# ka9q/ka9q-radio

Hardware: NVIDIA H100
Metric: input Msamples/s through forward+filter+inverse at N channels (higher is better)
Workload: dtype f32

## Files before the change

include/ka9q_gpu.h:

```cpp
#ifndef KA9Q_GPU_H
#define KA9Q_GPU_H 1
#include <stddef.h>
#include <stdint.h>

#ifdef __cplusplus
extern "C" {
#endif

enum kgpu_type { KGPU_COMPLEX = 1, KGPU_REAL = 2 };
enum kgpu_format {
  KGPU_FMT_F32 = 0,
  KGPU_FMT_I16 = 1
};
enum kgpu_chan_flags {
  KGPU_CHAN_ISB = 1,
  KGPU_CHAN_BEAM = 4
};

typedef struct kgpu_master kgpu_master;
typedef struct kgpu_bank kgpu_bank;

struct kgpu_ingest_stats {
  unsigned long long energy;
  unsigned int clips;
// ... 132 lines not shown
long kgpu_bank_out_offset(kgpu_bank const *b, int idx);
int kgpu_bank_run(kgpu_bank *b, const void *d_spec, int nblocks, void *d_out, void *stream);
int kgpu_bank_run_ex(kgpu_bank *b, const void *d_spec, int nblocks, void *d_out, long out_pitch, float *d_power, void *stream);
int kgpu_bank_run_one(kgpu_bank *b, int idx, const void *d_spec, void *d_out, void *stream);
int kgpu_bank_run_one_ex(kgpu_bank *b, int idx, const void *d_spec, void *d_out, float *d_power , void *stream);
int kgpu_bank_noise(kgpu_bank *b, const void *d_spec, int nblocks, double samprate, double *d_n0, void *stream);

int kgpu_bank_fm_front(kgpu_bank *b, const void *d_out, long out_pitch, int nblocks, float *d_baseband, double *d_stats, void *stream);

int kgpu_bank_commit(kgpu_bank *b, void *stream);
int kgpu_use_static_kernels(int on);
int kgpu_use_cols_tma(int on);
int kgpu_cols_tma_fits(int L, int M, int in_type, int fmt, const void *d_in);
int kgpu_use_fused_forward(int on);
int kgpu_fused_forward_fits(int L, int M, int in_type, int fmt, const void *d_in);
int kgpu_fused_forward_options(int lead, int discard);
int kgpu_fused_shape(int *out);
int kgpu_fused_schedule(int nblocks, int lead, int ticket, int *out);
long kgpu_fused_discards(int blk, int idx, long *lines, long max);

int kgpu_plan_radices(int len, int *radices, int max);
int kgpu_plan_split(long n, int *n1, int *n2);
int kgpu_plan_radices_ex(int len, int *radices, int max);
int kgpu_plan_split_ex(long n, int *n1, int *n2);

int kgpu_multicast_copy(const void *d_src, void *mc_dst, unsigned long long bytes, int nctas, void *stream);

typedef struct kgpu_spectrum kgpu_spectrum;
kgpu_spectrum *kgpu_spectrum_create(int fft_n, int in_type, int bin_count);
int kgpu_spectrum_set_window(kgpu_spectrum *s, float const *window);
int kgpu_spectrum_run(kgpu_spectrum *s, const void *d_ring, long ring_samples, long end, int fmt, float scale,
                      const struct kgpu_scale_change *d_chg, int nchg, long long end_index, int derandomize, int shift, int fft_avg, double overlap, float *d_bins, void *stream);
int kgpu_spectrum_run_narrow(kgpu_spectrum *s, const void *d_ring, long ring_size, long ring_idx, int fft_avg,
                             double overlap, float *d_bins, int *fft_avg_used, void *stream);
// ... 12 lines not shown
```

ka9q_radio_b200/capi.py:

```python
from __future__ import annotations

import ctypes as C
import os
import subprocess
from pathlib import Path

PKG = Path(__file__).resolve().parent
LIB_PATH = PKG / "libka9qgpu.so"

KGPU_COMPLEX, KGPU_REAL = 1, 2
KGPU_FMT_F32, KGPU_FMT_I16 = 0, 1
KGPU_RAW_U8, KGPU_RAW_S8 = 1, 2
KGPU_RAW_S16, KGPU_RAW_U16, KGPU_RAW_SC16Q11 = 3, 4, 5
KGPU_RAW_F32, KGPU_RAW_CF32, KGPU_RAW_CF32_CNRMF, KGPU_RAW_CF32_FSCALE = 6, 7, 8, 9
KGPU_CHAN_ISB = 1
KGPU_CHAN_BEAM = 4

_lib = None


class KgpuError(RuntimeError):
    pass


# ... 81 lines not shown
    L.kgpu_bank_block_counter.restype = l
    L.kgpu_bank_run_ex.argtypes = [vp, vp, i, vp, l, vp, vp]
    L.kgpu_bank_run_one_ex.argtypes = [vp, i, vp, vp, vp, vp]
    L.kgpu_bank_noise.argtypes = [vp, vp, i, d, vp, vp]
    L.kgpu_bank_fm_front.argtypes = [vp, vp, l, i, vp, vp, vp]
    L.kgpu_use_static_kernels.argtypes = [i]
    L.kgpu_use_cols_tma.argtypes = [i]
    L.kgpu_cols_tma_fits.argtypes = [i, i, i, i, vp]
    L.kgpu_use_fused_forward.argtypes = [i]
    L.kgpu_fused_forward_fits.argtypes = [i, i, i, i, vp]
    L.kgpu_fused_forward_options.argtypes = [i, i]
    L.kgpu_fused_shape.argtypes = [vp]
    L.kgpu_fused_schedule.argtypes = [i, i, i, vp]
    L.kgpu_fused_discards.argtypes = [i, i, vp, l]
    L.kgpu_fused_discards.restype = l
    L.kgpu_profile_enable.argtypes = [i]
    L.kgpu_profile_name.argtypes = [i]
    L.kgpu_profile_name.restype = C.c_char_p
    L.kgpu_profile_get.argtypes = [i, vp, vp]
    L.kgpu_plan_radices.argtypes = [i, vp, i]
    L.kgpu_plan_split.argtypes = [l, vp, vp]
    L.kgpu_plan_radices_ex.argtypes = [i, vp, i]
    L.kgpu_plan_split_ex.argtypes = [l, vp, vp]
    L.kgpu_multicast_copy.argtypes = [vp, vp, C.c_ulonglong, i, vp]
    L.kgpu_algorithmic_bytes.argtypes = [vp, vp, i]
    L.kgpu_algorithmic_bytes.restype = d
    L.kgpu_spectrum_create.restype = vp
    L.kgpu_spectrum_create.argtypes = [i, i, i]
    L.kgpu_spectrum_set_window.argtypes = [vp, vp]
    L.kgpu_spectrum_run.argtypes = [vp, vp, l, l, i, f, vp, i, C.c_longlong, i, i, i, d, vp, vp]
# ... 369 lines not shown
```

ka9q_radio_b200/csrc/fft_static.cuh:

```cuda
#pragma once
#include "fft_radix.cuh"

namespace kfft {

template <int LEN, int... RS> struct SPlan {
  static constexpr int len = LEN;
  static constexpr int nst = sizeof...(RS);
  static constexpr int rad_arr[sizeof...(RS) > 0 ? sizeof...(RS) : 1] = {RS...};
  static constexpr int rad(int i) { return rad_arr[i]; }
  static constexpr int nsub(int i) {
    int n = LEN;
    for (int k = 0; k < i; k++) n /= rad_arr[k];
    return n;
  }
  static constexpr int stride(int i) { return nsub(i) / rad_arr[i]; }
  static constexpr int tw_off(int i) {
    int o = 0;
    for (int k = 0; k < i; k++)
      if (stride(k) > 1) o += (rad_arr[k] - 1) * stride(k);
    return o;
  }
  static constexpr bool valid() {
    int p = 1;
    for (int k = 0; k < nst; k++) p *= rad_arr[k];
// ... 99 lines not shown
};

__device__ __forceinline__ uint32_t smem_u32(void const *p) { return (uint32_t)__cvta_generic_to_shared(p); }
__device__ __forceinline__ void mbar_init(uint64_t *bar, int count) {
  asm volatile("mbarrier.init.shared::cta.b64 [%0], %1;" ::"r"(smem_u32(bar)), "r"(count));
}
__device__ __forceinline__ void mbar_fence_init() { asm volatile("fence.mbarrier_init.release.cluster;" ::: "memory"); }
__device__ __forceinline__ void mbar_expect_tx(uint64_t *bar, uint32_t bytes) {
  asm volatile("mbarrier.arrive.expect_tx.shared::cta.b64 _, [%0], %1;" ::"r"(smem_u32(bar)), "r"(bytes) : "memory");
}
__device__ __forceinline__ void bulk_g2s(void *dst, void const *src, uint32_t bytes, uint64_t *bar) {
  asm volatile("cp.async.bulk.shared::cluster.global.mbarrier::complete_tx::bytes [%0], [%1], %2, [%3];" ::"r"(smem_u32(dst)),
               "l"(src), "r"(bytes), "r"(smem_u32(bar))
               : "memory");
}
__device__ __forceinline__ void tensor_g2s_3d(void *dst, void const *map, int x, int y, int z, uint64_t *bar) {
  asm volatile("cp.async.bulk.tensor.3d.shared::cluster.global.tile.mbarrier::complete_tx::bytes [%0], [%1, {%2, %3, %4}], [%5];"
               ::"r"(smem_u32(dst)), "l"(map), "r"(x), "r"(y), "r"(z), "r"(smem_u32(bar))
               : "memory");
}
__device__ __forceinline__ void fence_proxy_async_global() { asm volatile("fence.proxy.async.global;" ::: "memory"); }
__device__ __forceinline__ void discard_l2_line(void *p) { asm volatile("discard.global.L2 [%0], 128;" ::"l"(p) : "memory"); }
__device__ __forceinline__ void mbar_wait(uint64_t *bar, uint32_t parity) {
  asm volatile(
      "{\n\t.reg .pred p;\n\t"
      "WAIT_%=:\n\t"
      "mbarrier.try_wait.parity.shared::cta.b64 p, [%0], %1;\n\t"
      "@p bra DONE_%=;\n\t"
      "bra WAIT_%=;\n\t"
      "DONE_%=:\n\t}" ::"r"(smem_u32(bar)),
// ... 6 lines not shown
```

ka9q_radio_b200/csrc/fwd_fused.cuh:

```cuda
#pragma once
#include "fwd_cols_r36.cuh"
#include "static_kernels_v2.cuh"

namespace kfft {

struct FusedShape {
  static constexpr int N1 = 1296, N2 = 1250;
  static constexpr int TILES = (N2 + 7) / 8;
  static constexpr int NC = (TILES + 1) / 2;
  static constexpr int NR = (N1 / 2 + 1 + RowsV2Shape<true>::IPC - 1) / RowsV2Shape<true>::IPC;
  static constexpr int T = 2 * ColsR36Shape::T;
  static constexpr int RT = RowsV2Shape<true>::T;
  static constexpr size_t smem = 2 * ColsR36Shape::smem > RowsV2Shape<true>::smem ? 2 * ColsR36Shape::smem : RowsV2Shape<true>::smem;
  static constexpr int DEFAULT_LEAD = 40;
  static_assert(ColsR36Shape::smem % 16 == 0, "the second tile's memory 16-byte aligned");
  static_assert(T % 32 == 0 && ColsR36Shape::T % 32 == 0 && RT % 32 == 0, "whole warps per tile and per R item");
};

enum FusedKind : int { kFusedCol = 0, kFusedRow = 1 };
struct FusedItem {
  int kind, blk, idx;
};

__host__ __device__ __forceinline__ FusedItem fused_item(int t, int nblocks, int lead) {
// ... 12 lines not shown
  unsigned *ctr;
  int nblocks, lead;
  int discard;
};

__device__ __forceinline__ void red_release_gpu_add(unsigned *p, unsigned v) {
  asm volatile("red.release.gpu.global.add.u32 [%0], %1;" ::"l"(p), "r"(v) : "memory");
}
__device__ __forceinline__ unsigned ld_acquire_gpu(unsigned const *p) {
  unsigned v;
  asm volatile("ld.acquire.gpu.global.u32 %0, [%1];" : "=r"(v) : "l"(p) : "memory");
  return v;
}

template <int FMT>
__global__ void __launch_bounds__(FusedShape::T, 1)
    fwd_fused_r36_v2(Pass1Args const a1, ColsR36Tables const t1, Pass2Args const a2, FwdTables const t2, FusedArgs const f,
                     const __grid_constant__ CUtensorMap tmap) {
  using F = FusedShape;
  extern __shared__ __align__(16) unsigned char smem_raw[];
  __shared__ __align__(8) uint64_t bars[RowsV2Shape<true>::COLS];
  __shared__ __align__(8) uint64_t tbar[2];
  __shared__ int s_ticket;
  int const tid = threadIdx.x;
  if (tid == 0) s_ticket = (int)atomicAdd(f.ctr, 1u);
  __syncthreads();
  FusedItem const it = fused_item(s_ticket, f.nblocks, f.lead);
  if (it.kind == kFusedCol) {
    int const h = tid >= ColsR36Shape::T, tile = 2 * it.idx + h;
    if (tile < F::TILES)
      fwd_cols_r36_body<FMT, F::N2, true>(a1, t1, &tmap, smem_raw + h * ColsR36Shape::smem, tbar[h], tid - h * ColsR36Shape::T,
                                           tile * 8, it.blk, [h] {
                                             asm volatile("bar.sync %0, %1;" ::"r"(1 + h), "n"(ColsR36Shape::T) : "memory");
                                           });
    __syncthreads();
    if (tid == 0) {
      __threadfence();
      red_release_gpu_add(f.ctr + 1 + fused_item(s_ticket, f.nblocks, f.lead).blk, 1u);
    }
    return;
  }
  if (tid >= F::RT) return;
  auto sync = [] { asm volatile("bar.sync 3, %0;" ::"n"(F::RT) : "memory"); };
  auto sync_or = [](int p) {
    int r;
    asm volatile("{\n\t.reg .pred q, o;\n\tsetp.ne.s32 q, %1, 0;\n\tbar.red.or.pred o, 3, %2, q;\n\tselp.s32 %0, 1, 0, o;\n\t}"
                 : "=r"(r)
                 : "r"(p), "n"(F::RT)
                 : "memory");
    return r;
  };
  if (tid == 0)
    while (ld_acquire_gpu(f.ctr + 1 + it.blk) < (unsigned)F::NC) __nanosleep(64);
  sync();
  fwd_rows_v2_body<true, F::N1, true, true>(a2, t2, smem_raw, bars, tbar[0], tid, it.blk, it.idx * RowsV2Shape<true>::IPC,
                                            sync, sync_or, f.discard);
}

}
```

ka9q_radio_b200/csrc/kgpu.cu:

```cuda
#include <cuda_runtime.h>
#include <cudaTypedefs.h>
#include <math.h>
#include <stdarg.h>
#include <stdio.h>
#include <stdlib.h>
#include <string.h>
#include <algorithm>
#include <complex>
#include <atomic>
#include <map>
#include <mutex>
#include <string>
#include <vector>

#include "../../include/ka9q_gpu.h"
#include "chan_kernels.cuh"
#include "chan_huge.cuh"
#include "chan_wide.cuh"
#include "fwd_kernels.cuh"
#include "noise_kernel.cuh"
#include "plan.cuh"
#include "static_kernels.cuh"
#include "static_kernels_v2.cuh"
#include "fwd_cols_r36.cuh"
// ... 19 lines not shown
static std::atomic<int> g_cols_tma{-1};
extern "C" int kgpu_use_cols_tma(int on) {
  g_cols_tma.store(on != 0);
  return 0;
}
static bool cols_tma_on() {
  int v = g_cols_tma.load();
  if (v < 0) {
    char const *e = getenv("KA9Q_COLS_TMA");
    g_cols_tma.compare_exchange_strong(v, (e && *e) ? (atoi(e) != 0) : 1);
    v = g_cols_tma.load();
  }
  return v != 0;
}
static std::atomic<int> g_fused{-1};
static std::atomic<int> g_fused_lead{FusedShape::DEFAULT_LEAD}, g_fused_discard{0};
extern "C" int kgpu_use_fused_forward(int on) {
  g_fused.store(on != 0);
  return 0;
}
static bool fused_on() {
  int v = g_fused.load();
  if (v < 0) {
    char const *e = getenv("KA9Q_FUSED_FWD");
    g_fused.compare_exchange_strong(v, (e && *e) ? (atoi(e) != 0) : 1);
    v = g_fused.load();
  }
  return v != 0;
}

static int fail(char const *fmt, ...) {
  char buf[512];
  va_list ap;
  va_start(ap, fmt);
  vsnprintf(buf, sizeof buf, fmt, ap);
  va_end(ap);
  g_err = buf;
  return -1;
}
#define CUDA_OK(expr)                                                                    \
  do {                                                                                   \
    cudaError_t e_ = (expr);                                                             \
    if (e_ != cudaSuccess) return fail("%s: %s (%s:%d)", #expr, cudaGetErrorString(e_), __FILE__, __LINE__); \
// ... 921 lines not shown
  return k[f];
}
static RowsV2Fn rows_v2_kernel(kgpu_master const *m) {
  if (m->in_type == KGPU_REAL) return m->halved ? fwd_rows_v2<true, 1296, true> : fwd_rows_v2<true, 0, false>;
  return m->n1c ? fwd_rows_v2<false, 1296, false> : fwd_rows_v2<false, 0, false>;
}
static bool fused_pair(kgpu_master const *m) {
  return m->in_type == KGPU_REAL && m->cols == COLS_R36 && m->rows == ROWS_V2 && m->halved && m->n2c == FusedShape::N2 &&
         m->n1c == FusedShape::N1 && m->mid_ld % 16 == 0;
}
using FusedFn = void (*)(Pass1Args, ColsR36Tables, Pass2Args, FwdTables, FusedArgs, CUtensorMap);
static FusedFn fused_kernel(int f) {
  static FusedFn const k[3] = {fwd_fused_r36_v2<0>, fwd_fused_r36_v2<1>, fwd_fused_r36_v2<2>};
  return k[f];
}
static int rows_v2_threads(kgpu_master const *m) { return m->in_type == KGPU_REAL ? RowsV2Shape<true>::T : RowsV2Shape<false>::T; }
static size_t rows_v2_smem(kgpu_master const *m) {
  return m->in_type == KGPU_REAL ? RowsV2Shape<true>::smem : RowsV2Shape<false>::smem;
}

static int upload(float2 **d, std::vector<float2> const &v) {
  CUDA_OK(cudaMalloc(d, sizeof(float2) * v.size()));
  CUDA_OK(cudaMemcpy(*d, v.data(), sizeof(float2) * v.size(), cudaMemcpyHostToDevice));
  return 0;
}

static int bluestein_upload(Bluestein *b) {
  if (upload(&b->d_b, bluestein_bspec(b->n, b->P)) == 0) return 0;
  cudaFree(b->d_b);
  b->d_b = nullptr;
// ... 84 lines not shown
      for (int j = 0; j < RB; j++) t0[(size_t)e * RB + j] = root((long)j * Pow<RA>::exponent(e), n1);
    for (long c = 0; c < n2; c++) {
      for (int t = 0; t < RA; t++) tA[(size_t)c * RA + t] = root(c * t, m->nc);
      for (int e = 0; e < Cols2s::NP1; e++) tB[(size_t)c * Cols2s::NP1 + e] = root(c * RA * Pow<RB>::exponent(e), m->nc);
    }
    for (int e = 0; e < Rows2s::NP0; e++)
      for (int j = 0; j < RD; j++) r0[(size_t)e * RD + j] = root((long)j * Pow<RC>::exponent(e), n2);
    if (upload(&m->d_tw0, t0) || upload(&m->d_twA, tA) || upload(&m->d_twB, tB) || upload(&m->d_rtw0, r0)) return -1;
    for (int f = 0; f < 3; f++)
      if (allow_smem((const void *)cols_2s_kernel(f), Cols2s::smem)) return -1;
    if (allow_smem((const void *)fwd_rows_2s<25, 25>, Rows2s::smem)) return -1;
  }
  if (m->rows == ROWS_V2 && allow_smem((const void *)rows_v2_kernel(m), rows_v2_smem(m))) return -1;
  if (fused_pair(m))
    for (int f = 0; f < 3; f++)
      if (allow_smem((const void *)fused_kernel(f), FusedShape::smem)) return -1;
  if (m->ext) {
    if (allow_smem((const void *)fwd_cols_ext<0>, m->smem1) || allow_smem((const void *)fwd_cols_ext<1>, m->smem1) ||
        allow_smem((const void *)fwd_rows_ext, m->smem2))
      return -1;
  } else if (allow_smem((const void *)fwd_cols_kernel<0>, m->smem1) || allow_smem((const void *)fwd_cols_kernel<1>, m->smem1) ||
             allow_smem((const void *)fwd_rows_kernel, m->smem2)) {
    return -1;
  }
  return 0;
}

extern "C" void kgpu_master_destroy(kgpu_master *m) {
  if (!m) return;
  if (m->ext) {
    free_tile_plan(m->xplan1);
// ... 193 lines not shown
  MasterPlan pl;
  if (master_plan(L, M, in_type, MP_BLUESTEIN, "kgpu_fused_forward_fits", &pl)) return -1;
  if (pl.path != MP_DIRECT) return 0;
  kgpu_master m;
  master_shape(&m, L, M, in_type, pl.sp, false);
  return fused_fits(&m, d_in, fmt) ? 1 : 0;
}

extern "C" int kgpu_fused_forward_options(int lead, int discard) {
  if (lead < 0 || lead > FusedShape::NC) return fail("kgpu_fused_forward_options: lead %d outside 0..%d", lead, FusedShape::NC);
  g_fused_lead.store(lead);
  g_fused_discard.store(discard != 0);
  return 0;
}

extern "C" int kgpu_fused_shape(int *out) {
  if (!out) return fail("kgpu_fused_shape: bad arguments");
  out[0] = FusedShape::NC;
  out[1] = FusedShape::NR;
  out[2] = FusedShape::N1;
  out[3] = (FusedShape::N2 + 15) / 16 * 16;
  out[4] = FusedShape::DEFAULT_LEAD;
  return 0;
}

extern "C" int kgpu_fused_schedule(int nblocks, int lead, int ticket, int *out) {
  if (nblocks < 1 || lead < 0 || lead > FusedShape::NC || ticket < 0 || ticket >= nblocks * (FusedShape::NC + FusedShape::NR) ||
      !out)
    return fail("kgpu_fused_schedule: bad arguments");
  FusedItem const it = fused_item(ticket, nblocks, lead);
  out[0] = it.kind;
  out[1] = it.blk;
  out[2] = it.idx;
  out[3] = it.kind == kFusedRow ? it.blk : -1;
  out[4] = it.kind == kFusedRow ? FusedShape::NC : 0;
  return 0;
}

extern "C" long kgpu_fused_discards(int blk, int idx, long *lines, long max) {
  using S = RowsV2Shape<true>;
  if (blk < 0 || idx < 0 || idx >= FusedShape::NR || max < 0) return fail("kgpu_fused_discards: bad arguments");
  int const ld = (FusedShape::N2 + 15) / 16 * 16;
  long n = 0;
  for (int col = 0; col < S::COLS; col++) {
    RowItem const it = row_item(idx * S::IPC + (col >> 1), FusedShape::N1, true);
    int const row = (col & 1) == 0 ? (it.kind != kRowEmpty ? it.row_a : -1) : (it.kind == kRowPair ? it.row_b : -1);
    if (row < 0) continue;
    for (int l = 0; l < mid_row_lines(ld); l++, n++)
      if (lines && n < max) lines[n] = mid_line(blk, FusedShape::N1, row, ld, l);
  }
  return n;
// ... 30 lines not shown
  a2.n2 = m->sp.n2;
  a2.nc = m->nc;
  a2.plan = m->plan2;
  a2.pitch = m->pitch2;
  a2.real_split = (m->in_type == KGPU_REAL);
  a2.rootD = m->d_rootD;
  a2.spec = (float2 *)d_spec;
  a2.spec_stride = m->spec_stride;
  a2.mid_ld = a1.mid_ld;
  return a2;
}

static int fused_span(kgpu_master *m, const void *d_in, int fmt, int f, int nblocks, void *d_spec, cudaStream_t st,
                      Pass1Args const &a1) {
  using F = FusedShape;
  size_t const ctr_bytes = sizeof(unsigned) * (size_t)(1 + nblocks);
  if (grow(m->fused_ctr, ctr_bytes, st, "kgpu_forward")) return -1;
  CUtensorMap map;
  if (cols_tma_map(m, d_in, fmt, nblocks, &map)) return -1;
  FusedArgs fa;
  fa.ctr = (unsigned *)m->fused_ctr.p;
  fa.nblocks = nblocks;
  fa.lead = g_fused_lead.load();
  fa.discard = g_fused_discard.load();
  CUDA_OK(cudaMemsetAsync(fa.ctr, 0, ctr_bytes, st));
  {
    ProfScope ps(K_FWD_FUSED, st);
    fused_kernel(f)<<<(unsigned)(nblocks * (F::NC + F::NR)), F::T, F::smem, st>>>(a1, ColsR36Tables{m->d_tw0, m->d_twA, m->d_twB},
                                                                       rows_args(m, a1, d_spec), FwdTables{m->d_rootC}, fa, map);
  }
  g_launches++;
  CUDA_OK(cudaGetLastError());
  return 0;
}

static int forward_span(kgpu_master *m, const void *d_in, int fmt, float scale, int derandomize, int nblocks, void *d_spec,
                        void *d_stats, cudaStream_t st, float2 *mid) {
  bool const use_static = g_static_on.load() != 0;
  ColsKernel const cols = use_static ? m->cols : COLS_GENERIC;
  RowsKernel const rows = use_static ? m->rows : ROWS_GENERIC;
  Pass1Args a1;
  a1.in = d_in;
  a1.hop = (m->in_type == KGPU_REAL) ? m->L / 2 : m->L;
  a1.n1 = m->sp.n1;
// ... 1399 lines not shown
```

ka9q_radio_b200/csrc/static_kernels_v2.cuh:

```cuda
#pragma once
#include "static_kernels.cuh"

namespace kfft {

__device__ __forceinline__ void unpack_i16(int raw, int &lo, int &hi) {
  asm("prmt.b32 %0, %1, 0, 0x9910;" : "=r"(lo) : "r"(raw));
  hi = raw >> 16;
}
__device__ __forceinline__ float i32_to_f32(int v) {
  float f;
  asm("cvt.rn.f32.s32 %0, %1;" : "=f"(f) : "r"(v));
  return f;
}

template <bool REAL_SPLIT>
struct RowsV2Shape {
  using P = SPlan<1250, 10, 25, 5>;
  static constexpr int N2 = 1250, PITCH = 1250, GT = 256, SKEW = 2;
  static constexpr int NG = REAL_SPLIT ? 2 : 1, T = GT * NG, COLS = 8 * NG;
  static constexpr int IPC = REAL_SPLIT ? COLS / 2 : COLS;
  static constexpr int TW = (static_tw_count<P>() + 1) & ~1;
  static constexpr int TILE = COLS * PITCH + (NG - 1) * SKEW;
  static constexpr size_t smem = sizeof(float2) * (size_t)(TILE + TW);
  static __host__ __device__ constexpr int col_off(int c) { return c * PITCH + (c >> 3) * SKEW; }
};

__device__ constexpr float kRowsTw0[3][4][2] = {
    {{9.870916009e-01f, -1.601568460e-01f}, {9.486995935e-01f, -3.161789477e-01f}, {8.000617623e-01f, -5.999176502e-01f}, {2.801976204e-01f, -9.599423409e-01f}},
    {{9.486995935e-01f, -3.161789477e-01f}, {8.000617623e-01f, -5.999176502e-01f}, {2.801976204e-01f, -9.599423409e-01f}, {-8.429785967e-01f, -5.379471183e-01f}},
    {{8.858151436e-01f, -4.640382826e-01f}, {5.693368912e-01f, -8.221042752e-01f}, {-3.517109454e-01f, -9.361086488e-01f}, {-7.525988221e-01f, 6.584793329e-01f}},
};

__host__ __device__ constexpr int mid_row_lines(int mid_ld) { return mid_ld * 8 / 128; }
__host__ __device__ constexpr long mid_line(int blk, int n1, int row, int mid_ld, int l) {
  return ((long)blk * n1 + row) * mid_row_lines(mid_ld) + l;
}

template <bool REAL_SPLIT, int N1C, bool HALVED, bool FUSED, class Sync, class SyncOr>
__device__ __forceinline__ void fwd_rows_v2_body(Pass2Args const &a, FwdTables const &tb, unsigned char *smem_raw,
                                                 uint64_t *bars, uint64_t &tbar, int tid, int blk, int item0,
                                                 Sync const &sync, SyncOr const &sync_or, bool discard = false) {
  using S = RowsV2Shape<REAL_SPLIT>;
  using P = typename S::P;
  constexpr int N2 = S::N2, T = S::T, GT = S::GT, COLS = S::COLS, IPC = S::IPC;
  constexpr int R0 = 10, S0 = 125, R1 = 25, NSUB1 = 125, S1 = 5, R2 = 5;
  float2 *tile = reinterpret_cast<float2 *>(smem_raw);
  float2 *s_tw = tile + S::TILE;
  TilePlan const &pl = c_plans[a.plan];
  int const lane = tid & 31, warp = tid >> 5;
  int const n1 = N1C ? N1C : a.n1;
  auto row_of = [&](int col) -> int {
    RowItem const it = row_item(item0 + (REAL_SPLIT ? col >> 1 : col), n1, REAL_SPLIT);
    if (REAL_SPLIT) {
      if ((col & 1) == 0) return it.kind != kRowEmpty ? it.row_a : -1;
      return it.kind == kRowPair ? it.row_b : -1;
    }
    return it.kind == kRowPlain ? it.row_a : -1;
  };
  if (lane == 0) {
    int const row = row_of(warp);
// ... 14 lines not shown
  sync();
  int const g = tid / GT;
  int const c = (tid & 7) + 8 * g, ul = (tid % GT) >> 3;
  auto group_sync = [&] {
    if (S::NG == 1) sync();
    else asm volatile("bar.sync %0, %1;" ::"r"(1 + g), "n"(GT) : "memory");
  };
  bool const col_ok = row_of(c) >= 0;
  mbar_wait(&tbar, 0);
  if (col_ok) mbar_wait(&bars[c], 0);
  if (FUSED && discard && col_ok) {
    char *const mid = const_cast<char *>(reinterpret_cast<char const *>(a.mid));
    for (int l = ul; l < mid_row_lines(a.mid_ld); l += GT / 8) discard_l2_line(mid + 128 * mid_line(blk, n1, row_of(c), a.mid_ld, l));
  }
  float2 *mycol = tile + S::col_off(c);

  if (col_ok) {
    float2 base[4];
#pragma unroll
    for (int q = 0; q < 4; q++) base[q] = s_tw[((1 << q) - 1) * S0 + ul];
#pragma unroll
    for (int it = 0; it < 4; it++) {
      int const j = ul + (GT / 8) * it;
      if (it < 3 || j < S0) {
        float2 *p = mycol + j;
        float2 x[R0], w[R0];
#pragma unroll
        for (int m = 0; m < R0; m++) x[m] = p[m * S0];
#pragma unroll
        for (int q = 0; q < 4; q++)
          w[1 << q] = it == 0 ? base[q] : cmul(base[q], make_float2(kRowsTw0[it > 0 ? it - 1 : 0][q][0], kRowsTw0[it > 0 ? it - 1 : 0][q][1]));
        w[3] = cmul(w[2], w[1]);
        w[5] = cmul(w[4], w[1]);
        w[6] = cmul(w[4], w[2]);
        w[7] = cmul(w[4], w[3]);
        w[9] = cmul(w[8], w[1]);
        Dft<R0, false>::run(x);
        p[0] = x[0];
#pragma unroll
        for (int t = 1; t < R0; t++) p[t * S0] = cmul(x[t], w[t]);
      }
    }
  }
  group_sync();
  if (col_ok) {
    float2 const *tw1 = s_tw + P::tw_off(1);
#pragma unroll 1
    for (int u = ul; u < N2 / R1; u += GT / 8) {
      int const b = u / S1, j = u - b * S1;
      float2 *p = mycol + b * NSUB1 + j;
      float2 x[R1];
#pragma unroll
      for (int m = 0; m < R1; m++) x[m] = p[m * S1];
      Dft<R1, false>::run(x);
#pragma unroll
      for (int t = 1; t < R1; t++) x[t] = cmul(x[t], tw1[(t - 1) * S1 + j]);
#pragma unroll
      for (int t = 0; t < R1; t++) p[t * S1] = x[t];
    }
  }
  constexpr int UQ = T / IPC;
  int const i = tid % IPC, uq = tid / IPC;
  RowItem const it = row_item(item0 + i, n1, REAL_SPLIT);
  float2 rootC = make_float2(1.f, 0.f), rd[4];
  bool self_item = false;
  if (REAL_SPLIT) {
    self_item = it.kind == kRowSelf0 || it.kind == kRowSelfMid;
    if (it.kind == kRowPair) rootC = __ldg(tb.rootC + it.row_a);
#pragma unroll
    for (int q = 0; q < 4; q++) {
      int const u = uq + UQ * q;
      int const t0 = u / 25, t1 = u - t0 * 25;
      rd[q] = (it.kind == kRowPair && u < N2 / R2) ? __ldg(a.rootD + t0 + 10 * t1) : make_float2(1.f, 0.f);
    }
  }
  int const has_self = sync_or(self_item);

  float2 *spec = a.spec + (long)blk * a.spec_stride;
  float const hf = HALVED ? 1.0f : 0.5f;
  if (!REAL_SPLIT) {
    if (col_ok) {
      float2 *dst = spec + row_of(c);
#pragma unroll 1
      for (int u = ul; u < N2 / R2; u += GT / 8) {
        int const t0 = u / 25, t1 = u - t0 * 25;
        int const kb = t0 + 10 * t1;
        float2 const *p = mycol + u * R2;
        float2 x[R2];
#pragma unroll
        for (int m = 0; m < R2; m++) x[m] = p[m];
        Dft<R2, false>::run(x);
        float2 *d = dst + (long)n1 * kb;
#pragma unroll
        for (int t = 0; t < R2; t++) d[(long)n1 * 250 * t] = x[t];
// ... 16 lines not shown
      float2 *pk = spec + (it.row_a + n1 * kb), *pm = spec + (nc - it.row_a - n1 * kb);
#pragma unroll
      for (int m = 0; m < R2; m++) {
        za[m] = pa[m];
        zb[m] = pb[m];
      }
      Dft<R2, false>::run(za);
      Dft<R2, false>::run(zb);
#pragma unroll
      for (int t = 0; t < R2; t++) {
        float2 const A = za[t], B = zb[R2 - 1 - t];
        float2 const w = (t == 0) ? wkb : cmul(wkb, wroot<10>(t));
        float2 const E = HALVED ? make_float2(A.x + B.x, A.y - B.y) : make_float2(0.5f * (A.x + B.x), 0.5f * (A.y - B.y));
        float2 const O = HALVED ? make_float2(A.x - B.x, A.y + B.y) : make_float2(0.5f * (A.x - B.x), 0.5f * (A.y + B.y));
        float2 const Pp = cmul(w, O);
        pk[(long)n1 * 250 * t] = make_float2(E.x + Pp.y, E.y - Pp.x);
        pm[-(long)n1 * 250 * t] = make_float2(E.x - Pp.y, -(E.y + Pp.x));
      }
    }
  }
  if (!has_self) return;
  for (int s = 0; s < IPC; s++) {
    RowItem const its = row_item(item0 + s, n1, true);
    if (its.kind != kRowSelf0 && its.kind != kRowSelfMid) continue;
    float2 *col = tile + S::col_off(2 * s);
    for (int u = tid; u < N2 / R2; u += T) {
      float2 x[R2];
#pragma unroll
      for (int m = 0; m < R2; m++) x[m] = col[u * R2 + m];
      Dft<R2, false>::run(x);
#pragma unroll
      for (int m = 0; m < R2; m++) col[u * R2 + m] = x[m];
// ... 3 lines not shown
  for (int s = 0; s < IPC; s++) {
    RowItem const its = row_item(item0 + s, n1, true);
    if (its.kind != kRowSelf0 && its.kind != kRowSelfMid) continue;
    float2 const *col = tile + S::col_off(2 * s);
    float2 const rC = __ldg(tb.rootC + its.row_a);
    bool const self0 = its.kind == kRowSelf0;
    int const kend = self0 ? N2 / 2 + 1 : (N2 + 1) / 2;
    for (int k2 = tid; k2 < kend; k2 += T) {
      int const k2m = self0 ? (k2 == 0 ? 0 : N2 - k2) : N2 - 1 - k2;
      float2 const A = col[static_slot<P>(k2)], B = col[static_slot<P>(k2m)];
      float2 const w = cmul(rC, __ldg(a.rootD + k2));
      float2 const E = make_float2(hf * (A.x + B.x), hf * (A.y - B.y));
      float2 const O = make_float2(hf * (A.x - B.x), hf * (A.y + B.y));
      float2 const Pp = cmul(w, O);
      int const k = its.row_a + n1 * k2;
      spec[k] = make_float2(E.x + Pp.y, E.y - Pp.x);
      if (nc - k != k) spec[nc - k] = make_float2(E.x - Pp.y, -(E.y + Pp.x));
    }
  }
}

template <bool REAL_SPLIT, int N1C = 0, bool HALVED = false>
__global__ void __launch_bounds__(RowsV2Shape<REAL_SPLIT>::T, REAL_SPLIT ? 1 : 2) fwd_rows_v2(Pass2Args const a, FwdTables const tb) {
  extern __shared__ __align__(16) unsigned char smem_raw[];
  __shared__ __align__(8) uint64_t bars[RowsV2Shape<REAL_SPLIT>::COLS];
  __shared__ __align__(8) uint64_t tbar;
  fwd_rows_v2_body<REAL_SPLIT, N1C, HALVED, false>(a, tb, smem_raw, bars, tbar, threadIdx.x, gridDim.y - 1 - blockIdx.y,
                                                   blockIdx.x * RowsV2Shape<REAL_SPLIT>::IPC, [] { __syncthreads(); },
                                                   [](int p) { return __syncthreads_or(p); });
}

template <class P, bool OSC = false>
// ... 62 lines not shown
```

Baseline: 104,100.

## Add three-phase fused forward FFT with separate row and split work items

Adds a v3 fused forward kernel that schedules column tiles, row-FFT groups that write their results back to the mid buffer via bulk shared-to-global copies, and separate real-split tiles that combine mirrored rows into the spectrum. The intent is to decouple the real-split postprocessing from the row FFTs and spread it over more CTAs, improving load balance and overlap in the persistent ticket schedule. It also switches fused spectrum stores to streaming stores and enables L2 discard by default. In exchange, each mid row takes an extra global round trip and there are additional inter-CTA dependency counters and spin waits.

```diff
diff --git a/include/ka9q_gpu.h b/include/ka9q_gpu.h
--- a/include/ka9q_gpu.h
+++ b/include/ka9q_gpu.h
@@ -170,10 +170,15 @@
 int kgpu_cols_tma_fits(int L, int M, int in_type, int fmt, const void *d_in);
 int kgpu_use_fused_forward(int on);
 int kgpu_fused_forward_fits(int L, int M, int in_type, int fmt, const void *d_in);
+int kgpu_fused_forward_form(int form);
 int kgpu_fused_forward_options(int lead, int discard);
 int kgpu_fused_shape(int *out);
 int kgpu_fused_schedule(int nblocks, int lead, int ticket, int *out);
 long kgpu_fused_discards(int blk, int idx, long *lines, long max);
+int kgpu_fused3_shape(int *out);
+int kgpu_fused3_schedule(int nblocks, int lead, int ticket, int *out);
+int kgpu_fused3_rows(int blk, int idx, long *out);
+long kgpu_fused3_bins(int idx, long *bins, long max);
 
 int kgpu_plan_radices(int len, int *radices, int max);
 int kgpu_plan_split(long n, int *n1, int *n2);
diff --git a/ka9q_radio_b200/capi.py b/ka9q_radio_b200/capi.py
--- a/ka9q_radio_b200/capi.py
+++ b/ka9q_radio_b200/capi.py
@@ -119,6 +119,12 @@
     L.kgpu_fused_schedule.argtypes = [i, i, i, vp]
     L.kgpu_fused_discards.argtypes = [i, i, vp, l]
     L.kgpu_fused_discards.restype = l
+    L.kgpu_fused_forward_form.argtypes = [i]
+    L.kgpu_fused3_shape.argtypes = [vp]
+    L.kgpu_fused3_schedule.argtypes = [i, i, i, vp]
+    L.kgpu_fused3_rows.argtypes = [i, i, vp]
+    L.kgpu_fused3_bins.argtypes = [i, vp, l]
+    L.kgpu_fused3_bins.restype = l
     L.kgpu_profile_enable.argtypes = [i]
     L.kgpu_profile_name.argtypes = [i]
     L.kgpu_profile_name.restype = C.c_char_p
diff --git a/ka9q_radio_b200/csrc/fft_static.cuh b/ka9q_radio_b200/csrc/fft_static.cuh
--- a/ka9q_radio_b200/csrc/fft_static.cuh
+++ b/ka9q_radio_b200/csrc/fft_static.cuh
@@ -137,6 +137,13 @@
                "l"(src), "r"(bytes), "r"(smem_u32(bar))
                : "memory");
 }
+__device__ __forceinline__ void bulk_s2g(void *dst, void const *src, uint32_t bytes) {
+  asm volatile("cp.async.bulk.global.shared::cta.bulk_group [%0], [%1], %2;" ::"l"(dst), "r"(smem_u32(src)), "r"(bytes) : "memory");
+}
+__device__ __forceinline__ void bulk_s2g_wait() {
+  asm volatile("cp.async.bulk.commit_group;\n\tcp.async.bulk.wait_group 0;" ::: "memory");
+}
+__device__ __forceinline__ void fence_proxy_async_shared() { asm volatile("fence.proxy.async.shared::cta;" ::: "memory"); }
 __device__ __forceinline__ void tensor_g2s_3d(void *dst, void const *map, int x, int y, int z, uint64_t *bar) {
   asm volatile("cp.async.bulk.tensor.3d.shared::cluster.global.tile.mbarrier::complete_tx::bytes [%0], [%1, {%2, %3, %4}], [%5];"
                ::"r"(smem_u32(dst)), "l"(map), "r"(x), "r"(y), "r"(z), "r"(smem_u32(bar))
diff --git a/ka9q_radio_b200/csrc/fwd_fused.cuh b/ka9q_radio_b200/csrc/fwd_fused.cuh
--- a/ka9q_radio_b200/csrc/fwd_fused.cuh
+++ b/ka9q_radio_b200/csrc/fwd_fused.cuh
@@ -50,6 +50,19 @@
 }
 
 template <int FMT>
+__device__ __forceinline__ void fused_col_item(Pass1Args const &a1, ColsR36Tables const &t1, CUtensorMap const *tmap,
+                                               unsigned char *smem_raw, uint64_t *tbar, int tid, int blk, int idx) {
+  using F = FusedShape;
+  int const h = tid >= ColsR36Shape::T, tile = 2 * idx + h;
+  if (tile < F::TILES)
+    fwd_cols_r36_body<FMT, F::N2, true>(a1, t1, tmap, smem_raw + h * ColsR36Shape::smem, tbar[h], tid - h * ColsR36Shape::T,
+                                         tile * 8, blk, [h] {
+                                           asm volatile("bar.sync %0, %1;" ::"r"(1 + h), "n"(ColsR36Shape::T) : "memory");
+                                         });
+  __syncthreads();
+}
+
+template <int FMT>
 __global__ void __launch_bounds__(FusedShape::T, 1)
     fwd_fused_r36_v2(Pass1Args const a1, ColsR36Tables const t1, Pass2Args const a2, FwdTables const t2, FusedArgs const f,
                      const __grid_constant__ CUtensorMap tmap) {
@@ -63,13 +76,7 @@
   __syncthreads();
   FusedItem const it = fused_item(s_ticket, f.nblocks, f.lead);
   if (it.kind == kFusedCol) {
-    int const h = tid >= ColsR36Shape::T, tile = 2 * it.idx + h;
-    if (tile < F::TILES)
-      fwd_cols_r36_body<FMT, F::N2, true>(a1, t1, &tmap, smem_raw + h * ColsR36Shape::smem, tbar[h], tid - h * ColsR36Shape::T,
-                                           tile * 8, it.blk, [h] {
-                                             asm volatile("bar.sync %0, %1;" ::"r"(1 + h), "n"(ColsR36Shape::T) : "memory");
-                                           });
-    __syncthreads();
+    fused_col_item<FMT>(a1, t1, &tmap, smem_raw, tbar, tid, it.blk, it.idx);
     if (tid == 0) {
       __threadfence();
       red_release_gpu_add(f.ctr + 1 + fused_item(s_ticket, f.nblocks, f.lead).blk, 1u);
@@ -93,4 +100,207 @@
                                             sync, sync_or, f.discard);
 }
 
-}
+struct Fused3Shape {
+  using F = FusedShape;
+  static constexpr int N1 = F::N1, N2 = F::N2, NC = F::NC;
+  static constexpr int RR = 16;
+  static constexpr int NR = N1 / RR;
+  static constexpr int SPLIT = 626;
+  static constexpr int NS = 2 * NR;
+  static constexpr int SUB = 128, NSUB = (SPLIT + SUB - 1) / SUB;
+  static constexpr int SP = SUB + 2;
+  static constexpr size_t s_smem = sizeof(float2) * ((size_t)NSUB * 2 * RR * SP + N2);
+  static constexpr size_t smem = F::smem > s_smem ? F::smem : s_smem;
+  static constexpr int DEFAULT_LEAD = NC;
+  static __host__ __device__ constexpr int slot_of(int k2) { return 5 * (25 * (k2 % 10) + (k2 % 250) / 10) + k2 / 250; }
+  static __host__ __device__ constexpr int k2_of(int slot) { return (slot / 5) / 25 + 10 * ((slot / 5) % 25) + 250 * (slot % 5); }
+  static_assert(N1 % RR == 0 && N1 % 16 == 0, "whole row groups; 16 k1 = 128 bytes from a 32-byte aligned base");
+  static_assert(SPLIT % 2 == 0 && SUB % 2 == 0 && SP % 16 == 2, "bulk copies of 16-byte multiples at 16-byte offsets");
+  static_assert((N2 - SPLIT + SUB - 1) / SUB == NSUB, "both S tiles have NSUB sub-tiles");
+  static_assert(F::T / 32 >= NSUB, "a warp per sub-tile's copies");
+  static_assert(RowsV2Shape<true>::COLS == RR && RowsV2Shape<true>::T <= F::T, "an R item is fwd_rows_v2's REAL tile");
+};
+enum : int { kFusedSplit = 2 };
+struct Fused3Tile {
+  int k1_0, s0, s1;
+};
+__host__ __device__ __forceinline__ Fused3Tile fused3_tile(int idx) {
+  using G = Fused3Shape;
+  return {G::RR * (idx >> 1), (idx & 1) ? G::SPLIT : 0, (idx & 1) ? G::N2 : G::SPLIT};
+}
+__host__ __device__ __forceinline__ long fused3_row(int blk, int y, int c, int mid_ld) {
+  return ((long)blk * Fused3Shape::N1 + Fused3Shape::RR * y + c) * mid_ld;
+}
+
+__host__ __device__ __forceinline__ FusedItem fused3_item(int t, int nblocks, int lead) {
+  using G = Fused3Shape;
+  if (t < G::NC) return {kFusedCol, 0, t};
+  t -= G::NC;
+  int b = 0, nc, nr;
+  for (;; b++) {
+    nc = b + 1 < nblocks ? G::NC : 0;
+    nr = b < nblocks ? G::NR : 0;
+    int const len = nc + nr + (b >= 1 ? G::NS : 0);
+    if (t < len) break;
+    t -= len;
+  }
+  if (t >= nc + nr) return {kFusedSplit, b - 1, t - nc - nr};
+  int const ld = lead < nc ? lead : nc;
+  if (t < ld) return {kFusedCol, b + 1, t};
+  int const q = t - ld, m = nc - ld < nr ? nc - ld : nr;
+  if (q < 2 * m) return (q & 1) ? FusedItem{kFusedCol, b + 1, ld + q / 2} : FusedItem{kFusedRow, b, q / 2};
+  return nc - ld > nr ? FusedItem{kFusedCol, b + 1, ld + q - m} : FusedItem{kFusedRow, b, q - m};
+}
+
+template <class Sync>
+__device__ __forceinline__ void fused3_rows_body(Pass2Args const &a, unsigned char *smem_raw, uint64_t *bars, uint64_t &tbar,
+                                                 int tid, int blk, int y, Sync const &sync) {
+  using S = RowsV2Shape<true>;
+  constexpr int N2 = S::N2, GT = S::GT, R2 = 5;
+  float2 *tile = reinterpret_cast<float2 *>(smem_raw);
+  float2 *s_tw = tile + S::TILE;
+  int const lane = tid & 31, warp = tid >> 5;
+  float2 *const zt = const_cast<float2 *>(a.mid) + fused3_row(blk, y, warp, a.mid_ld);
+  if (lane == 0) {
+    mbar_init(&bars[warp], 1);
+    if (warp == 0) mbar_init(&tbar, 1);
+    mbar_fence_init();
+    fence_proxy_async_global();
+    mbar_expect_tx(&bars[warp], N2 * 8);
+    bulk_g2s(tile + S::col_off(warp), zt, N2 * 8, &bars[warp]);
+    if (warp == 0) {
+      constexpr uint32_t TWB = (uint32_t)S::TW * 8u;
+      mbar_expect_tx(&tbar, TWB);
+      bulk_g2s(s_tw, c_plans[a.plan].tw, TWB, &tbar);
+    }
+  }
+  sync();
+  int const g = tid / GT, c = (tid & 7) + 8 * g, ul = (tid % GT) >> 3;
+  auto group_sync = [&] { asm volatile("bar.sync %0, %1;" ::"r"(1 + g), "n"(GT) : "memory"); };
+  mbar_wait(&tbar, 0);
+  mbar_wait(&bars[c], 0);
+  float2 *mycol = tile + S::col_off(c);
+  rows_v2_stages01<S>(mycol, s_tw, ul, true, group_sync);
+  group_sync();
+#pragma unroll 1
+  for (int u = ul; u < N2 / R2; u += GT / 8) {
+    float2 *p = mycol + u * R2;
+    float2 x[R2];
+#pragma unroll
+    for (int m = 0; m < R2; m++) x[m] = p[m];
+    Dft<R2, false>::run(x);
+#pragma unroll
+    for (int m = 0; m < R2; m++) p[m] = x[m];
+  }
+  fence_proxy_async_shared();
+  group_sync();
+  if (lane == 0) {
+    bulk_s2g(zt, tile + S::col_off(warp), N2 * 8);
+    bulk_s2g_wait();
+    fence_proxy_async_global();
+  }
+  sync();
+}
+
+__device__ __forceinline__ void fused3_split_body(Pass2Args const &a, FwdTables const &tb, unsigned char *smem_raw,
+                                                  uint64_t *bars, int tid, int blk, int idx) {
+  using G = Fused3Shape;
+  constexpr int N1 = G::N1, N2 = G::N2, H = N1 / 2, RR = G::RR, SP = G::SP, SUB = G::SUB, NW = FusedShape::T / 32;
+  float2 *const buf = reinterpret_cast<float2 *>(smem_raw);
+  float2 *const row0 = buf + G::NSUB * 2 * RR * SP;
+  Fused3Tile const tl = fused3_tile(idx);
+  int const s0 = tl.s0, s1 = tl.s1;
+  int const lane = tid & 31, warp = tid >> 5;
+  float2 const *const zt = a.mid + (long)blk * N1 * a.mid_ld;
+  if (warp < G::NSUB) {
+    int const lo = s0 + SUB * warp, w = min(SUB, s1 - lo);
+    if (lane == 0) {
+      mbar_init(&bars[warp], 1);
+      mbar_fence_init();
+      mbar_expect_tx(&bars[warp], (uint32_t)((2 * RR - (tl.k1_0 == 0)) * w * 8 + (tl.k1_0 == 0 && warp == 0 ? N2 * 8 : 0)));
+    }
+    __syncwarp();
+    int const k1 = tl.k1_0 + (lane & (RR - 1));
+    float2 *const dst = buf + (warp * 2 * RR + lane) * SP;
+    fence_proxy_async_global();
+    if (lane < RR) bulk_g2s(dst, zt + (long)k1 * a.mid_ld + lo, w * 8, &bars[warp]);
+    else if (k1 != 0) bulk_g2s(dst, zt + (long)(N1 - k1) * a.mid_ld + (N2 - lo - w), w * 8, &bars[warp]);
+    else if (warp == 0) bulk_g2s(row0, zt, N2 * 8, &bars[0]);
+  }
+  __syncthreads();
+  int const i = (lane & 7) + 8 * (lane >> 4), par = (lane >> 3) & 1, k1 = tl.k1_0 + i;
+  bool const self = k1 == 0 || k1 == H;
+  float2 const rC = __ldg(tb.rootC + (k1 <= H ? k1 : N1 - k1));
+  float2 *const spec = a.spec + (long)blk * a.spec_stride;
+#pragma unroll 1
+  for (int s = 0; s < G::NSUB; s++) {
+    int const lo = s0 + SUB * s, w = min(SUB, s1 - lo);
+    float2 const *const zs = buf + (s * 2 * RR + i) * SP, *const zp = zs + RR * SP;
+    mbar_wait(&bars[s], 0);
+#pragma unroll 1
+    for (int q = 2 * warp + par; q < w; q += 2 * NW) {
+      int const k2 = G::k2_of(lo + q);
+      float2 const z = zs[q];
+      float2 const y = k1 != 0 ? zp[w - 1 - q] : row0[G::slot_of(k2 == 0 ? 0 : N2 - k2)];
+      bool const low = !self ? k1 < H : k2 <= (k1 == 0 ? N2 / 2 : N2 / 2 - 1);
+      float2 const A = low ? z : y, B = low ? y : z;
+      int const ka = low ? k2 : (k1 == 0 ? N2 - k2 : N2 - 1 - k2);
+      float2 wv;
+      if (!self) {
+        int const t = ka / 250;
+        float2 const wkb = cmul(rC, __ldg(a.rootD + (ka - 250 * t)));
+        wv = t == 0 ? wkb : cmul(wkb, wroot<10>(t));
+      } else {
+        wv = cmul(rC, __ldg(a.rootD + ka));
+      }
+      float2 const E = make_float2(A.x + B.x, A.y - B.y);
+      float2 const O = make_float2(A.x - B.x, A.y + B.y);
+      float2 const Pp = cmul(wv, O);
+      spec[k1 + (long)N1 * k2] = low ? make_float2(E.x + Pp.y, E.y - Pp.x) : make_float2(E.x - Pp.y, -(E.y + Pp.x));
+      if (k1 == 0 && k2 == 0) spec[(long)N1 * N2] = make_float2(E.x - Pp.y, -(E.y + Pp.x));
+    }
+  }
+}
+
+template <int FMT>
+__global__ void __launch_bounds__(FusedShape::T, 1)
+    fwd_fused_r36_v3(Pass1Args const a1, ColsR36Tables const t1, Pass2Args const a2, FwdTables const t2, FusedArgs const f,
+                     const __grid_constant__ CUtensorMap tmap) {
+  using F = FusedShape;
+  using G = Fused3Shape;
+  extern __shared__ __align__(16) unsigned char smem_raw[];
+  __shared__ __align__(8) uint64_t bars[RowsV2Shape<true>::COLS];
+  __shared__ __align__(8) uint64_t tbar[2];
+  __shared__ int s_ticket;
+  int const tid = threadIdx.x;
+  if (tid == 0) s_ticket = (int)atomicAdd(f.ctr, 1u);
+  __syncthreads();
+  FusedItem const it = fused3_item(s_ticket, f.nblocks, f.lead);
+  if (it.kind == kFusedCol) {
+    fused_col_item<FMT>(a1, t1, &tmap, smem_raw, tbar, tid, it.blk, it.idx);
+    if (tid == 0) {
+      __threadfence();
+      red_release_gpu_add(f.ctr + 1 + fused3_item(s_ticket, f.nblocks, f.lead).blk, 1u);
+    }
+    return;
+  }
+  if (it.kind == kFusedRow) {
+    if (tid >= F::RT) return;
+    auto sync = [] { asm volatile("bar.sync 3, %0;" ::"n"(F::RT) : "memory"); };
+    if (tid == 0)
+      while (ld_acquire_gpu(f.ctr + 1 + it.blk) < (unsigned)G::NC) __nanosleep(64);
+    sync();
+    fused3_rows_body(a2, smem_raw, bars, tbar[0], tid, it.blk, it.idx, sync);
+    if (tid == 0) {
+      __threadfence();
+      red_release_gpu_add(f.ctr + 1 + f.nblocks + it.blk, 1u);
+    }
+    return;
+  }
+  if (tid == 0)
+    while (ld_acquire_gpu(f.ctr + 1 + f.nblocks + it.blk) < (unsigned)G::NR) __nanosleep(64);
+  __syncthreads();
+  fused3_split_body(a2, t2, smem_raw, bars, tid, it.blk, it.idx);
+}
+
+}
diff --git a/ka9q_radio_b200/csrc/kgpu.cu b/ka9q_radio_b200/csrc/kgpu.cu
--- a/ka9q_radio_b200/csrc/kgpu.cu
+++ b/ka9q_radio_b200/csrc/kgpu.cu
@@ -57,7 +57,9 @@
   return v != 0;
 }
 static std::atomic<int> g_fused{-1};
-static std::atomic<int> g_fused_lead{FusedShape::DEFAULT_LEAD}, g_fused_discard{0};
+static std::atomic<int> g_fused_lead{-1}, g_fused_discard{1};
+static constexpr int kFusedFormDefault = 2;
+static std::atomic<int> g_fused_form{-1};
 extern "C" int kgpu_use_fused_forward(int on) {
   g_fused.store(on != 0);
   return 0;
@@ -70,6 +72,16 @@
     v = g_fused.load();
   }
   return v != 0;
+}
+static int fused_form() {
+  int v = g_fused_form.load();
+  if (v < 0) {
+    char const *e = getenv("KA9Q_FUSED_FORM");
+    int const want = (e && *e) ? atoi(e) : kFusedFormDefault;
+    g_fused_form.compare_exchange_strong(v, want == 2 || want == 3 ? want : kFusedFormDefault);
+    v = g_fused_form.load();
+  }
+  return v;
 }
 
 static int fail(char const *fmt, ...) {
@@ -1021,6 +1033,10 @@
   static FusedFn const k[3] = {fwd_fused_r36_v2<0>, fwd_fused_r36_v2<1>, fwd_fused_r36_v2<2>};
   return k[f];
 }
+static FusedFn fused3_kernel(int f) {
+  static FusedFn const k[3] = {fwd_fused_r36_v3<0>, fwd_fused_r36_v3<1>, fwd_fused_r36_v3<2>};
+  return k[f];
+}
 static int rows_v2_threads(kgpu_master const *m) { return m->in_type == KGPU_REAL ? RowsV2Shape<true>::T : RowsV2Shape<false>::T; }
 static size_t rows_v2_smem(kgpu_master const *m) {
   return m->in_type == KGPU_REAL ? RowsV2Shape<true>::smem : RowsV2Shape<false>::smem;
@@ -1135,7 +1151,8 @@
   if (m->rows == ROWS_V2 && allow_smem((const void *)rows_v2_kernel(m), rows_v2_smem(m))) return -1;
   if (fused_pair(m))
     for (int f = 0; f < 3; f++)
-      if (allow_smem((const void *)fused_kernel(f), FusedShape::smem)) return -1;
+      if (allow_smem((const void *)fused_kernel(f), FusedShape::smem) || allow_smem((const void *)fused3_kernel(f), Fused3Shape::smem))
+        return -1;
   if (m->ext) {
     if (allow_smem((const void *)fwd_cols_ext<0>, m->smem1) || allow_smem((const void *)fwd_cols_ext<1>, m->smem1) ||
         allow_smem((const void *)fwd_rows_ext, m->smem2))
@@ -1359,6 +1376,12 @@
   return 0;
 }
 
+extern "C" int kgpu_fused_forward_form(int form) {
+  if (form != 2 && form != 3) return fail("kgpu_fused_forward_form: form %d is neither 2 nor 3", form);
+  g_fused_form.store(form);
+  return 0;
+}
+
 extern "C" int kgpu_fused_shape(int *out) {
   if (!out) return fail("kgpu_fused_shape: bad arguments");
   out[0] = FusedShape::NC;
@@ -1380,6 +1403,52 @@
   out[3] = it.kind == kFusedRow ? it.blk : -1;
   out[4] = it.kind == kFusedRow ? FusedShape::NC : 0;
   return 0;
+}
+
+extern "C" int kgpu_fused3_shape(int *out) {
+  using G = Fused3Shape;
+  if (!out) return fail("kgpu_fused3_shape: bad arguments");
+  int const v[9] = {G::NC, G::NR, G::NS, G::N1, G::N2, (G::N2 + 15) / 16 * 16, G::RR, G::SPLIT, G::DEFAULT_LEAD};
+  for (int i = 0; i < 9; i++) out[i] = v[i];
+  return 0;
+}
+
+extern "C" int kgpu_fused3_schedule(int nblocks, int lead, int ticket, int *out) {
+  using G = Fused3Shape;
+  if (nblocks < 1 || lead < 0 || lead > G::NC || ticket < 0 || ticket >= nblocks * (G::NC + G::NR + G::NS) || !out)
+    return fail("kgpu_fused3_schedule: bad arguments");
+  FusedItem const it = fused3_item(ticket, nblocks, lead);
+  out[0] = it.kind;
+  out[1] = it.blk;
+  out[2] = it.idx;
+  out[3] = it.kind == kFusedRow ? 1 + it.blk : it.kind == kFusedSplit ? 1 + nblocks + it.blk : -1;
+  out[4] = it.kind == kFusedRow ? G::NC : it.kind == kFusedSplit ? G::NR : 0;
+  return 0;
+}
+
+extern "C" int kgpu_fused3_rows(int blk, int idx, long *out) {
+  using G = Fused3Shape;
+  if (blk < 0 || idx < 0 || idx >= G::NR || !out) return fail("kgpu_fused3_rows: bad arguments");
+  for (int c = 0; c < G::RR; c++) out[c] = fused3_row(blk, idx, c, (G::N2 + 15) / 16 * 16);
+  return 0;
+}
+
+extern "C" long kgpu_fused3_bins(int idx, long *bins, long max) {
+  using G = Fused3Shape;
+  if (idx < 0 || idx >= G::NS || max < 0) return fail("kgpu_fused3_bins: bad arguments");
+  Fused3Tile const tl = fused3_tile(idx);
+  long n = 0;
+  auto put = [&](long k) {
+    if (bins && n < max) bins[n] = k;
+    n++;
+  };
+  for (int slot = tl.s0; slot < tl.s1; slot++)
+    for (int i = 0; i < G::RR; i++) {
+      int const k1 = tl.k1_0 + i, k2 = G::k2_of(slot);
+      put(k1 + (long)G::N1 * k2);
+      if (k1 == 0 && k2 == 0) put((long)G::N1 * G::N2);
+    }
+  return n;
 }
 
 extern "C" long kgpu_fused_discards(int blk, int idx, long *lines, long max) {
@@ -1440,20 +1509,27 @@
 static int fused_span(kgpu_master *m, const void *d_in, int fmt, int f, int nblocks, void *d_spec, cudaStream_t st,
                       Pass1Args const &a1) {
   using F = FusedShape;
-  size_t const ctr_bytes = sizeof(unsigned) * (size_t)(1 + nblocks);
+  using G = Fused3Shape;
+  bool const v3 = fused_form() == 3;
+  size_t const ctr_bytes = sizeof(unsigned) * (size_t)(1 + (v3 ? 2 : 1) * nblocks);
   if (grow(m->fused_ctr, ctr_bytes, st, "kgpu_forward")) return -1;
   CUtensorMap map;
   if (cols_tma_map(m, d_in, fmt, nblocks, &map)) return -1;
   FusedArgs fa;
   fa.ctr = (unsigned *)m->fused_ctr.p;
   fa.nblocks = nblocks;
-  fa.lead = g_fused_lead.load();
+  int const lead = g_fused_lead.load();
+  fa.lead = lead >= 0 ? lead : v3 ? G::DEFAULT_LEAD : F::DEFAULT_LEAD;
   fa.discard = g_fused_discard.load();
   CUDA_OK(cudaMemsetAsync(fa.ctr, 0, ctr_bytes, st));
   {
     ProfScope ps(K_FWD_FUSED, st);
-    fused_kernel(f)<<<(unsigned)(nblocks * (F::NC + F::NR)), F::T, F::smem, st>>>(a1, ColsR36Tables{m->d_tw0, m->d_twA, m->d_twB},
-                                                                       rows_args(m, a1, d_spec), FwdTables{m->d_rootC}, fa, map);
+    if (v3)
+      fused3_kernel(f)<<<(unsigned)(nblocks * (G::NC + G::NR + G::NS)), F::T, G::smem, st>>>(
+          a1, ColsR36Tables{m->d_tw0, m->d_twA, m->d_twB}, rows_args(m, a1, d_spec), FwdTables{m->d_rootC}, fa, map);
+    else
+      fused_kernel(f)<<<(unsigned)(nblocks * (F::NC + F::NR)), F::T, F::smem, st>>>(a1, ColsR36Tables{m->d_tw0, m->d_twA, m->d_twB},
+                                                                         rows_args(m, a1, d_spec), FwdTables{m->d_rootC}, fa, map);
   }
   g_launches++;
   CUDA_OK(cudaGetLastError());
diff --git a/ka9q_radio_b200/csrc/static_kernels_v2.cuh b/ka9q_radio_b200/csrc/static_kernels_v2.cuh
--- a/ka9q_radio_b200/csrc/static_kernels_v2.cuh
+++ b/ka9q_radio_b200/csrc/static_kernels_v2.cuh
@@ -36,6 +36,57 @@
   return ((long)blk * n1 + row) * mid_row_lines(mid_ld) + l;
 }
 
+template <class S, class GroupSync>
+__device__ __forceinline__ void rows_v2_stages01(float2 *mycol, float2 const *s_tw, int ul, bool col_ok, GroupSync const &group_sync) {
+  using P = typename S::P;
+  constexpr int N2 = S::N2, GT = S::GT;
+  constexpr int R0 = 10, S0 = 125, R1 = 25, NSUB1 = 125, S1 = 5;
+  if (col_ok) {
+    float2 base[4];
+#pragma unroll
+    for (int q = 0; q < 4; q++) base[q] = s_tw[((1 << q) - 1) * S0 + ul];
+#pragma unroll
+    for (int it = 0; it < 4; it++) {
+      int const j = ul + (GT / 8) * it;
+      if (it < 3 || j < S0) {
+        float2 *p = mycol + j;
+        float2 x[R0], w[R0];
+#pragma unroll
+        for (int m = 0; m < R0; m++) x[m] = p[m * S0];
+#pragma unroll
+        for (int q = 0; q < 4; q++)
+          w[1 << q] = it == 0 ? base[q] : cmul(base[q], make_float2(kRowsTw0[it > 0 ? it - 1 : 0][q][0], kRowsTw0[it > 0 ? it - 1 : 0][q][1]));
+        w[3] = cmul(w[2], w[1]);
+        w[5] = cmul(w[4], w[1]);
+        w[6] = cmul(w[4], w[2]);
+        w[7] = cmul(w[4], w[3]);
+        w[9] = cmul(w[8], w[1]);
+        Dft<R0, false>::run(x);
+        p[0] = x[0];
+#pragma unroll
+        for (int t = 1; t < R0; t++) p[t * S0] = cmul(x[t], w[t]);
+      }
+    }
+  }
+  group_sync();
+  if (col_ok) {
+    float2 const *tw1 = s_tw + P::tw_off(1);
+#pragma unroll 1
+    for (int u = ul; u < N2 / R1; u += GT / 8) {
+      int const b = u / S1, j = u - b * S1;
+      float2 *p = mycol + b * NSUB1 + j;
+      float2 x[R1];
+#pragma unroll
+      for (int m = 0; m < R1; m++) x[m] = p[m * S1];
+      Dft<R1, false>::run(x);
+#pragma unroll
+      for (int t = 1; t < R1; t++) x[t] = cmul(x[t], tw1[(t - 1) * S1 + j]);
+#pragma unroll
+      for (int t = 0; t < R1; t++) p[t * S1] = x[t];
+    }
+  }
+}
+
 template <bool REAL_SPLIT, int N1C, bool HALVED, bool FUSED, class Sync, class SyncOr>
 __device__ __forceinline__ void fwd_rows_v2_body(Pass2Args const &a, FwdTables const &tb, unsigned char *smem_raw,
                                                  uint64_t *bars, uint64_t &tbar, int tid, int blk, int item0,
@@ -43,7 +94,7 @@
   using S = RowsV2Shape<REAL_SPLIT>;
   using P = typename S::P;
   constexpr int N2 = S::N2, T = S::T, GT = S::GT, COLS = S::COLS, IPC = S::IPC;
-  constexpr int R0 = 10, S0 = 125, R1 = 25, NSUB1 = 125, S1 = 5, R2 = 5;
+  constexpr int R2 = 5;
   float2 *tile = reinterpret_cast<float2 *>(smem_raw);
   float2 *s_tw = tile + S::TILE;
   TilePlan const &pl = c_plans[a.plan];
@@ -88,51 +139,7 @@
     for (int l = ul; l < mid_row_lines(a.mid_ld); l += GT / 8) discard_l2_line(mid + 128 * mid_line(blk, n1, row_of(c), a.mid_ld, l));
   }
   float2 *mycol = tile + S::col_off(c);
-
-  if (col_ok) {
-    float2 base[4];
-#pragma unroll
-    for (int q = 0; q < 4; q++) base[q] = s_tw[((1 << q) - 1) * S0 + ul];
-#pragma unroll
-    for (int it = 0; it < 4; it++) {
-      int const j = ul + (GT / 8) * it;
-      if (it < 3 || j < S0) {
-        float2 *p = mycol + j;
-        float2 x[R0], w[R0];
-#pragma unroll
-        for (int m = 0; m < R0; m++) x[m] = p[m * S0];
-#pragma unroll
-        for (int q = 0; q < 4; q++)
-          w[1 << q] = it == 0 ? base[q] : cmul(base[q], make_float2(kRowsTw0[it > 0 ? it - 1 : 0][q][0], kRowsTw0[it > 0 ? it - 1 : 0][q][1]));
-        w[3] = cmul(w[2], w[1]);
-        w[5] = cmul(w[4], w[1]);
-        w[6] = cmul(w[4], w[2]);
-        w[7] = cmul(w[4], w[3]);
-        w[9] = cmul(w[8], w[1]);
-        Dft<R0, false>::run(x);
-        p[0] = x[0];
-#pragma unroll
-        for (int t = 1; t < R0; t++) p[t * S0] = cmul(x[t], w[t]);
-      }
-    }
-  }
-  group_sync();
-  if (col_ok) {
-    float2 const *tw1 = s_tw + P::tw_off(1);
-#pragma unroll 1
-    for (int u = ul; u < N2 / R1; u += GT / 8) {
-      int const b = u / S1, j = u - b * S1;
-      float2 *p = mycol + b * NSUB1 + j;
-      float2 x[R1];
-#pragma unroll
-      for (int m = 0; m < R1; m++) x[m] = p[m * S1];
-      Dft<R1, false>::run(x);
-#pragma unroll
-      for (int t = 1; t < R1; t++) x[t] = cmul(x[t], tw1[(t - 1) * S1 + j]);
-#pragma unroll
-      for (int t = 0; t < R1; t++) p[t * S1] = x[t];
-    }
-  }
+  rows_v2_stages01<S>(mycol, s_tw, ul, col_ok, group_sync);
   constexpr int UQ = T / IPC;
   int const i = tid % IPC, uq = tid / IPC;
   RowItem const it = row_item(item0 + i, n1, REAL_SPLIT);
@@ -152,6 +159,10 @@
 
   float2 *spec = a.spec + (long)blk * a.spec_stride;
   float const hf = HALVED ? 1.0f : 0.5f;
+  auto put = [](float2 *p, float2 v) {
+    if (FUSED) __stcs(p, v);
+    else *p = v;
+  };
   if (!REAL_SPLIT) {
     if (col_ok) {
       float2 *dst = spec + row_of(c);
@@ -198,8 +209,8 @@
         float2 const E = HALVED ? make_float2(A.x + B.x, A.y - B.y) : make_float2(0.5f * (A.x + B.x), 0.5f * (A.y - B.y));
         float2 const O = HALVED ? make_float2(A.x - B.x, A.y + B.y) : make_float2(0.5f * (A.x - B.x), 0.5f * (A.y + B.y));
         float2 const Pp = cmul(w, O);
-        pk[(long)n1 * 250 * t] = make_float2(E.x + Pp.y, E.y - Pp.x);
-        pm[-(long)n1 * 250 * t] = make_float2(E.x - Pp.y, -(E.y + Pp.x));
+        put(pk + (long)n1 * 250 * t, make_float2(E.x + Pp.y, E.y - Pp.x));
+        put(pm - (long)n1 * 250 * t, make_float2(E.x - Pp.y, -(E.y + Pp.x)));
       }
     }
   }
@@ -233,8 +244,8 @@
       float2 const O = make_float2(hf * (A.x - B.x), hf * (A.y + B.y));
       float2 const Pp = cmul(w, O);
       int const k = its.row_a + n1 * k2;
-      spec[k] = make_float2(E.x + Pp.y, E.y - Pp.x);
-      if (nc - k != k) spec[nc - k] = make_float2(E.x - Pp.y, -(E.y + Pp.x));
+      put(spec + k, make_float2(E.x + Pp.y, E.y - Pp.x));
+      if (nc - k != k) put(spec + (nc - k), make_float2(E.x - Pp.y, -(E.y + Pp.x)));
     }
   }
 }
```

Result: faster. 106,000 (median of 6 runs) (+1.9%).
